# RuyiLian/CheckerPose

Measured on AMD Instinct MI355X. Metric: crops/sec forward (256x256, npt=512), higher is better.
Workload: dtype bf16; 1 GPU; LMO 'ape' hr18GNN2_res6_gnn3Skip_mlpQuery npt=512, PoseNet_GNNskip forward, deterministic random-init weights; global_batch=256, parallelism=dp1 (no forward collective), launch=hipGraph replay of 104 kernel launches

## Files before the change

checkerpose_amd/_abi.py:

```python
import ctypes as C
import os

_HERE = os.path.dirname(os.path.abspath(__file__))
LIB_PATH = os.environ.get("CHECKERPOSE_AMD_LIB") or os.path.join(_HERE, "libcheckerpose_hip.so")

CP_F32, CP_BF16, CP_F16 = 0, 1, 2
ACT_NONE, ACT_RELU, ACT_LEAKY = 0, 1, 2
LOSS_BCE, LOSS_L1 = 0, 1
POSE_ERR_ADD, POSE_ERR_ADI = 1, 2
BOP_ERR_MSSD, BOP_ERR_MSPD, BOP_ERR_PROJ, BOP_MAP_SMALL, BOP_MAP_LARGE = 1, 2, 4, 16, 32
BOP_MATCH_NO_LDS, BOP_MATCH_SCRATCH_MASK, BOP_SCORES_NO_LDS = 1, 2, 1


class CpConvDesc(C.Structure):
    _fields_ = [("dtype", C.c_int32), ("out_f32", C.c_int32), ("B", C.c_int32), ("H", C.c_int32), ("W", C.c_int32),
                ("Cin", C.c_int32), ("in_cstride", C.c_int32), ("in_coff", C.c_int32),
                ("R", C.c_int32), ("S", C.c_int32), ("stride", C.c_int32), ("pad", C.c_int32),
                ("Ho", C.c_int32), ("Wo", C.c_int32), ("Cout", C.c_int32), ("act", C.c_int32), ("slope", C.c_float), ("ksplit", C.c_int32),
                ("o_base", C.c_int64), ("o_sb", C.c_int64), ("o_sy", C.c_int64), ("o_sx", C.c_int64),
                ("o_sc", C.c_int64)]


_P, _I, _F, _L = C.c_void_p, C.c_int, C.c_float, C.c_longlong

# ... 71 lines not shown
    "cp_device_status": (_I, [_P, _I]),
    "cp_set_deterministic": (None, [_I]),
    "cp_get_deterministic": (_I, []),
    "cp_strerror": (C.c_char_p, [_I]),
    "cp_last_kernel": (C.c_char_p, []),
    "cp_kernel_log_begin": (None, []),
    "cp_kernel_log": (C.c_char_p, []),
    "cp_chan_align": (_I, [_I]),
    "cp_packed_weight_bytes": (C.c_size_t, [_I, _I, _I, _I, _I]),
    "cp_pack_conv_weight": (_I, [_P, _I, _P, _I, _I, _I, _I, _I, _I, _I, _P, _I, _P]),
    "cp_conv2d_igemm": (_I, [_P, C.POINTER(CpConvDesc), _P, _P, _P, _P, _P, _P]),
    "cp_conv2d_igemm_splitk": (_I, [_I, C.c_longlong, _I, _I]),
    "cp_packed_halo_weight_bytes": (C.c_size_t, [_I, _I, _I]),
    "cp_pack_conv3x3_halo_weight": (_I, [_P, _I, _P, _I, _I, _I, _P]),
    "cp_conv3x3_halo": (_I, [_P, C.POINTER(CpConvDesc), _P, _P, _P, _P, _P, _P]),
    "cp_conv2x2_halo_supported": (_I, [_I, _I, _I, _I]),
    "cp_packed_conv2x2_halo_weight_bytes": (C.c_size_t, [_I, _I, _I]),
    "cp_pack_conv2x2_halo_weight": (_I, [_P, _I, _P, _I, _I, _I, _P]),
    "cp_conv2x2_halo": (_I, [_P, C.POINTER(CpConvDesc), _P, _P, _P, _P, _P, _P]),
    "cp_conv3x3_s2_small_supported": (_I, [_I, _I, _I, _I]),
    "cp_conv3x3_s2_small_weight_bytes": (C.c_size_t, [_I, _I]),
    "cp_pack_conv3x3_s2_small_weight": (_I, [_P, _P, _I, _I, _I, _I, _P]),
    "cp_conv3x3_s2_small": (_I, [_P, C.POINTER(CpConvDesc), _P, _P, _P, _P, _P]),
    "cp_conv3x3_halo_up2x_supported": (_I, [_I, _I]),
    "cp_conv3x3_halo_up2x": (_I, [_P, C.POINTER(CpConvDesc), _P, _P, _P, _P, _P]),
    "cp_conv3x3_halo_seg_supported": (_I, [_I, _I, _I]),
    "cp_conv3x3_halo_seg": (_I, [_P, C.POINTER(CpConvDesc), _P, _P, _P, _P, _P, _P, _P, _I, _P]),
    "cp_pack_conv3x3_rows_weight": (_I, [_P, _I, _P, _I, _I, _I, _P]),
    "cp_basicblock_fused": (_I, [_P, C.POINTER(CpConvDesc), _P, _P, _P, _P, _P, _P, _P, _P]),
    "cp_bottleneck_fused": (_I, [_P, C.POINTER(CpConvDesc)] + [_P] * 14),
# ... 236 lines not shown
```

checkerpose_amd/csrc/api.hip:

```cpp
#include <stdarg.h>
#include <stdio.h>
#include <string.h>

#include "common.h"

extern "C" int cp_version(void) { return 218; }

std::atomic<int> g_cp_deterministic{0};
extern "C" void cp_set_deterministic(int on) { g_cp_deterministic.store(on ? 1 : 0, std::memory_order_relaxed); }
extern "C" int cp_get_deterministic(void) { return g_cp_deterministic.load(std::memory_order_relaxed); }

static std::atomic<uint32_t*> g_status_word[256];
uint32_t* cp_status_word(bool create) {
  const int dev = cp_current_device();
  if (dev < 0 || dev > 255) return nullptr;
  uint32_t* p = g_status_word[dev].load(std::memory_order_acquire);
  if (p || !create) return p;
  hipStreamCaptureStatus cs = hipStreamCaptureStatusNone;
  if (hipStreamIsCapturing(nullptr, &cs) == hipSuccess && cs != hipStreamCaptureStatusNone) return nullptr;
  uint32_t* q = nullptr;
  if (hipMalloc((void**)&q, 256) != hipSuccess) return nullptr;
  if (hipMemset(q, 0, 256) != hipSuccess) { (void)hipFree(q); return nullptr; }
  uint32_t* expect = nullptr;
  if (!g_status_word[dev].compare_exchange_strong(expect, q, std::memory_order_acq_rel)) { (void)hipFree(q); return expect; }
// ... 69 lines not shown
```

checkerpose_amd/csrc/conv3x3_halo.hip:

```cpp
#include <stdlib.h>

#include "common.h"
#include <cstring>

struct HaloParams {
  const void* in; const void* w; const float* scale; const float* shift; const void* res; void* out;
  int B, H, W, Cin, in_cs, in_coff, nchunk, Cout, ngroups, NB;
  int tiles_x, tiles_y, total_tiles;
  int act; float slope;
  uint32_t in_bytes, w_bytes;
  long long o_base, o_sb, o_sy, o_sx;
  int Hs, Ws; float up_sy, up_sx;
  const float* seg_w; const float* seg_b; float* seg_out; int seg_S;
};

constexpr int HTH = 8, HTW = 16, HPW = HTW + 2, HPH = HTH + 2, HNPIX = 192;
constexpr int HPLANE = HNPIX * 16, HBUF = 4 * HPLANE;
constexpr int USRH = 7, USRW = 11, USPIX = 80, USBUF = USPIX * 64;

template <typename Tag> struct MmaH;
template <> struct MmaH<F32Tag> {
  static __device__ __forceinline__ void run(const u32x4& w, const u32x4& a, f32x4& acc) {
    acc = __builtin_amdgcn_mfma_f32_16x16x4f32(__uint_as_float(w.x), __uint_as_float(a.x), acc, 0, 0, 0);
    acc = __builtin_amdgcn_mfma_f32_16x16x4f32(__uint_as_float(w.y), __uint_as_float(a.y), acc, 0, 0, 0);
// ... 518 lines not shown
  const int lane = (int)((i / E) % 64);
  size_t blk = i / (E * 64);
  const int nt = (int)(blk % 4); blk /= 4;
  const int tap = (int)(blk % 9); blk /= 9;
  const int c = (int)(blk % nchunk);
  const int g = (int)(blk / nchunk);
  const int row = lane & 15, kq = lane >> 4;
  const int n = g * 64 + (row >> 2) * 16 + nt * 4 + (row & 3);
  const int cin = c * (4 * E) + kq * E + e;
  float v = 0.f;
  if (n < Cout && cin < Cin) v = w[((size_t)n * Cin + cin) * 9 + tap];
  store_elem<Tag>(out, i, v);
}

static inline bool halo_wide(int Cout) { return Cout >= 256 && Cout % 256 == 0 && !cp_knob("CP_NO_HALO4"); }

template <typename Tag, int NT, int KS = 3>
__global__ __launch_bounds__(256) void conv3x3_halo_s_kernel(const HaloParams p) {
  if (KS == 2 && p.seg_S == CP_F16) cp_f16_saturate_on();
  constexpr int E = Tag::E;
  constexpr int KCH = 4 * E;
  constexpr int ES = 16 / E;
  constexpr int NTAP = KS * KS;
  constexpr int WPIECES = NTAP * NT * 64;
  constexpr int WITER = (WPIECES + 255) / 256;
  extern __shared__ __attribute__((aligned(16))) unsigned char smem[];
  unsigned char* const sA = smem;
  unsigned char* const sW = smem + HBUF;

  const int t = blockIdx.x;
// ... 632 lines not shown
    } else {
      if (residual) CP_LAUNCH((conv3x3_halo4_kernel<BF16Tag, true, false, false>), dim3(grid4), dim3(256), 2 * HBUF, st4, p);
      else CP_LAUNCH((conv3x3_halo4_kernel<BF16Tag, false, false, false>), dim3(grid4), dim3(256), 2 * HBUF, st4, p);
    }
    return cp_check_launch();
  }
  const unsigned grid = (unsigned)(((tt + 7) / 8) * 8 * p.NB);
  hipStream_t st = (hipStream_t)stream;
  if (d->dtype == CP_F32) {
    if (residual) CP_LAUNCH((conv3x3_halo_kernel<F32Tag, true>), dim3(grid), dim3(256), 2 * HBUF, st, p);
    else CP_LAUNCH((conv3x3_halo_kernel<F32Tag, false>), dim3(grid), dim3(256), 2 * HBUF, st, p);
  } else {
    if (residual) CP_LAUNCH((conv3x3_halo_kernel<BF16Tag, true>), dim3(grid), dim3(256), 2 * HBUF, st, p);
    else CP_LAUNCH((conv3x3_halo_kernel<BF16Tag, false>), dim3(grid), dim3(256), 2 * HBUF, st, p);
  }
  return cp_check_launch();
}

extern "C" int cp_conv3x3_halo_up2x_supported(int dtype, int Cout) {
  return (dtype == CP_F32 || dtype == CP_BF16) && halo_wide(Cout) ? 1 : 0;
}

extern "C" int cp_conv3x3_halo_up2x(cp_stream_t stream, const CpConvDesc* d, const void* in, const void* packed_w,
                                    const float* scale, const float* shift, void* out) {
  if (!d || !in || !packed_w || !scale || !shift || !out) return CP_ERR_INVALID;
  if (!cp_conv3x3_halo_up2x_supported(d->dtype, d->Cout) || !cp_act_ok(d->act, d->slope)) return CP_ERR_INVALID;
  if (d->R != 3 || d->S != 3 || d->stride != 1 || d->pad != 1 || d->Ho != d->H || d->Wo != d->W || d->out_f32 || d->o_sc != 1)
    return CP_ERR_INVALID;
  if (d->B <= 0 || d->H < 2 || d->W < 2 || (d->H & 1) || (d->W & 1)) return CP_ERR_INVALID;
  const int E = cp_chan_align(d->dtype), es = cp_elem_size(d->dtype);
// ... 196 lines not shown
```

checkerpose_amd/engine.py:

```python
import ctypes as C
import os

import torch

from . import _abi
from ._abi import ACT_LEAKY, ACT_NONE, ACT_RELU, CP_BF16, CP_F16, CP_F32, CpChainTail, CpChainTailConv, CpConvDesc, CpFuseConv

_TORCH_DT = {CP_F32: torch.float32, CP_BF16: torch.bfloat16}
USE_HALO = os.environ.get("CHECKERPOSE_AMD_HALO", "1") != "0"
USE_FUSED_BN = os.environ.get("CHECKERPOSE_AMD_FUSED_BN", "1") != "0"
USE_FUSED_BB = os.environ.get("CHECKERPOSE_AMD_FUSED_BB", "1") != "0"
USE_GEMM = os.environ.get("CHECKERPOSE_AMD_GEMM", "1") != "0"
USE_CHAIN = os.environ.get("CHECKERPOSE_AMD_CHAIN", "1") != "0"
USE_UP_FUSED = os.environ.get("CHECKERPOSE_AMD_UP_FUSED", "1") != "0"
USE_FUSE_OUT = os.environ.get("CHECKERPOSE_AMD_FUSE_OUT", "1") != "0"
USE_S2_SMALL = os.environ.get("CHECKERPOSE_AMD_S2_SMALL", "1") != "0"
USE_SEG_FUSED = os.environ.get("CHECKERPOSE_AMD_SEG_FUSED", "1") != "0"
USE_HALO2 = os.environ.get("CHECKERPOSE_AMD_HALO2", "1") != "0"
USE_CHAIN_TAILS = os.environ.get("CHECKERPOSE_AMD_CHAIN_TAILS", "1") != "0"
USE_CHAIN_TAIL = os.environ.get("CHECKERPOSE_AMD_CHAIN_TAIL", "1") != "0"
FUSE_OUT_MIN_BATCH = int(os.environ.get("CHECKERPOSE_AMD_FUSE_OUT_MIN_BATCH", "1"))
USE_MLP_FUSED = os.environ.get("CHECKERPOSE_AMD_MLP_FUSED", "1") != "0"
MLP_FUSED_MIN_ROWS = int(os.environ.get("CHECKERPOSE_AMD_MLP_FUSED_MIN_ROWS", "1"))
EDGE_SCHED = os.environ.get("CHECKERPOSE_AMD_EDGE_SCHED", "1") != "0"
USE_SPLITK = os.environ.get("CHECKERPOSE_AMD_SPLITK", "1") != "0"
GEMM_WS_SMALL_K = os.environ.get("CHECKERPOSE_AMD_GEMM_WS_SMALL_K", "1") != "0"
USE_MLP_GATHER = os.environ.get("CHECKERPOSE_AMD_MLP_GATHER", "1") != "0"
USE_PATCH_GATHER = os.environ.get("CHECKERPOSE_AMD_PATCH_GATHER", "1") != "0"
USE_STEM = os.environ.get("CHECKERPOSE_AMD_STEM", "1") != "0"
STEM_MIN_BATCH = int(os.environ.get("CHECKERPOSE_AMD_STEM_MIN_BATCH", "96"))
USE_EDGE_FUSED = os.environ.get("CHECKERPOSE_AMD_EDGE_FUSED", "1") != "0"
USE_GNN_F16 = os.environ.get("CHECKERPOSE_AMD_GNN_F16", "1") != "0"
# ... 258 lines not shown
            raise RuntimeError("conv %s: weight expects %d input channels, activation has %d" % (wkey, wCin, x.C))
        halo = (USE_HALO and R == 3 and S == 3 and stride == 1 and pad == 1 and ostr is None and not out_f32
                and not transposed and row_map is None and x.W >= 16 and x.H >= 8 and not (out_half or in_half))
        cdt = CP_F16 if in_half else self.dtype
        if halo and wCout <= 80 and self.dtype == CP_F32:
            halo = _rup(x.Cphys, 16) <= 1.15 * x.Cphys
        kmin = 16 * self.E if not (self.dtype == CP_BF16 and residual is None and x.B * x.H * x.W >= 16384 and GEMM_WS_SMALL_K) else 64
        gemm = (USE_GEMM and R == 1 and S == 1 and stride == 1 and pad == 0 and ostr is None and not out_f32
                and not transposed and row_map is None and wCout >= 96 and x.Cphys >= kmin and not out_half)
        s2small = (USE_S2_SMALL and self.dtype == CP_BF16 and R == 3 and S == 3 and stride == 2 and pad == 1 and ostr is None and not out_f32
                   and not transposed and row_map is None and residual is None and x.H % 2 == 0 and x.W % 2 == 0 and x.B >= self.chain_min
                   and not (out_half or in_half) and bool(self.lib.cp_conv3x3_s2_small_supported(x.H, x.W, x.Cphys, _rup(wCout, self.E))))
        halo2 = (USE_HALO2 and self.dtype == CP_BF16 and R == 2 and S == 2 and stride == 1 and pad == 1 and ostr is None and not out_f32
                 and not transposed and row_map is None and not in_half and not self.ws.repacks_every_step
                 and bool(self.lib.cp_conv2x2_halo_supported(self.dtype, x.H, x.W, _rup(wCout, self.E))))
        if (self.splitk and not transposed and row_map is None and (halo or gemm or s2small or halo2)
                and self.lib.cp_conv2d_igemm_splitk(cdt, x.B * ((x.H + 2 * pad - R) // stride + 1) * ((x.W + 2 * pad - S) // stride + 1),
                                                    R * S * x.Cphys, _rup(wCout, self.E))):
            halo = gemm = s2small = halo2 = False
        if s2small:
            ck = ("s2small", wkey, x.Cphys)
            if ck not in self.ws.cache:
                buf = torch.empty(self.lib.cp_conv3x3_s2_small_weight_bytes(x.Cphys, _rup(wCout, self.E)), dtype=torch.uint8, device=self.device)
                wc = w.contiguous()
                self.ws.keep.append(wc)
                st_ = torch.cuda.current_stream(self.device).cuda_stream
                _abi.check(self.lib.cp_pack_conv3x3_s2_small_weight(st_, wc.data_ptr(), wCout, wCin, x.Cphys, _rup(wCout, self.E), buf.data_ptr()),
                           "cp_pack_conv3x3_s2_small_weight(%s)" % wkey)
                self.ws.cache[ck] = buf
            packed = self.ws.cache[ck]
            halo = gemm = False
        elif halo2:
            ck = ("halo2", wkey, x.Cphys)
            if ck not in self.ws.cache:
                buf = torch.empty(self.lib.cp_packed_conv2x2_halo_weight_bytes(self.dtype, wCout, x.Cphys), dtype=torch.uint8, device=self.device)
                wc = w.contiguous()
                self.ws.keep.append(wc)
                st_ = torch.cuda.current_stream(self.device).cuda_stream
                _abi.check(self.lib.cp_pack_conv2x2_halo_weight(st_, self.dtype, wc.data_ptr(), wCout, wCin, x.Cphys, buf.data_ptr()),
                           "cp_pack_conv2x2_halo_weight(%s)" % wkey)
                self.ws.cache[ck] = buf
            packed = self.ws.cache[ck]
        elif halo:
            packed = self.ws.pack_halo(wkey, w, wCout, wCin, x.Cphys)
        elif gemm:
            packed = self.ws.pack_gemm(wkey, w, wCout, wCin, x.Cphys, **({"dtype": CP_F16} if in_half else {}))
        else:
            packed = self.ws.pack(wkey, w, wCout, wCin, R, S, x.Cphys, rows, transposed, phase, row_map, **({"dtype": CP_F16} if in_half else {}))
        sc, sh = self.ws.affine(wkey + "#" + str(phase), scale, shift, rows)
        Ho, Wo = out_hw if out_hw is not None else ((x.H + 2 * pad - R) // stride + 1, (x.W + 2 * pad - S) // stride + 1)
        d = CpConvDesc()
        d.dtype, d.out_f32 = (CP_F16 if in_half else self.dtype), (1 if out_f32 else (2 if out_half else 0))
        d.B, d.H, d.W = x.B, x.H, x.W
        d.Cin, d.in_cstride, d.in_coff = x.Cphys, x.cstride, x.coff
        d.R, d.S, d.stride, d.pad, d.Ho, d.Wo = R, S, stride, pad, Ho, Wo
        d.act, d.slope = act, slope
        d.ksplit = 0 if self.splitk else -1
        if ostr is None:
# ... 11 lines not shown
        if residual is not None and ostr is None:
            assert (residual.cstride, residual.coff, residual.H, residual.W) == (out.cstride, out.coff, out.H, out.W), \
                "residual must share the output layout"
        fn = self.lib.cp_conv3x3_halo if halo else (self.lib.cp_gemm_rows if gemm else self.lib.cp_conv2d_igemm)
        if halo2:
            fn = self.lib.cp_conv2x2_halo
        dref = C.byref(d)
        pw, ps, pt = packed.data_ptr(), sc.data_ptr(), sh.data_ptr()
        xtb = x.tbuf
        if halo:
            fam = "conv3x3_halo_s" if wCout <= 80 else ("conv3x3_halo4" if wCout % 256 == 0 else "conv3x3_halo")
        else:
            fam = "gemm_rows" if gemm else "conv_igemm"
        if halo2:
            fam = "conv3x3_halo_s"
        if s2small:
            fam = "conv3x3_s2_small"
            self._add(self.lib.cp_conv3x3_s2_small, lambda P: (dref, P(xtb), pw, ps, pt, P(otb)), fam + ":" + wkey, [xtb], [otb])
        else:
            self._add(fn, lambda P: (dref, P(xtb), pw, ps, pt, P(rtb) if rtb is not None else None, P(otb)),
                      fam + ":" + wkey, [xtb, rtb], [otb])
        fl = 2 * x.B * Ho * Wo * R * S * wCin * wCout
        self.flops += fl
        oes = 4 if out_f32 else self.es
        nbytes = (x.B * x.H * x.W * wCin * self.es + x.B * Ho * Wo * wCout * oes * (2 if residual is not None else 1)
                  + R * S * wCin * wCout * self.es)
        self.conv_log.append((wkey, x.B * Ho * Wo, wCout, R * S * wCin, fl, fam, nbytes))
        return out

    def would_splitk(self, M, K, Cout):
        return bool(self.splitk and self.lib.cp_conv2d_igemm_splitk(self.dtype, M, K, _rup(Cout, self.E)))
# ... 16 lines not shown
        d.B, d.H, d.W = x.B, Ho, Wo
        d.Cin, d.in_cstride, d.in_coff = x.Cphys, x.cstride, x.coff
        d.R, d.S, d.stride, d.pad, d.Ho, d.Wo = 3, 3, 1, 1, Ho, Wo
        d.act, d.slope, d.Cout = act, slope, out.Cphys
        d.o_base, d.o_sb, d.o_sy, d.o_sx, d.o_sc = out.coff, out.H * out.W * out.cstride, out.W * out.cstride, out.cstride, 1
        self.keep += [d, packed, sc, sh]
        fn = self.lib.cp_conv3x3_halo_up2x
        dref = C.byref(d)
        pw, ps, pt = packed.data_ptr(), sc.data_ptr(), sh.data_ptr()
        xtb, otb = x.tbuf, out.tbuf
        self._add(fn, lambda P: (dref, P(xtb), pw, ps, pt, P(otb)), "conv3x3_halo4:" + wkey, [xtb], [otb])
        fl = 2 * x.B * Ho * Wo * 9 * wCin * wCout
        self.flops += fl
        nbytes = x.B * x.H * x.W * wCin * self.es + x.B * Ho * Wo * wCout * self.es + 9 * wCin * wCout * self.es
        self.conv_log.append((wkey, x.B * Ho * Wo, wCout, 9 * wCin, fl, "conv3x3_halo4", nbytes))
        return out

    def can_conv_halo_seg(self, x: Act, Cout, S):
        return (USE_SEG_FUSED and USE_HALO and x.W >= 16 and x.H >= 8 and
                bool(self.lib.cp_conv3x3_halo_seg_supported(self.dtype, _rup(Cout, self.E), S)))

    def conv_halo_seg(self, x: Act, wkey, w, scale, shift, act, seg_key, seg_w, seg_b, seg_tbuf, slope=0.0):
        wCout, wCin = w.shape[0], w.shape[1]
        if wCin != x.C:
            raise RuntimeError("conv %s: weight expects %d input channels, activation has %d" % (wkey, wCin, x.C))
        packed = self.ws.pack_halo(wkey, w, wCout, wCin, x.Cphys)
        sc, sh = self.ws.affine(wkey + "#0", scale, shift, wCout)
        S = seg_w.shape[0]
        ck = ("seg_head", seg_key, self.dtype)
        if ck not in self.ws.cache:
# ... 813 lines not shown
```

checkerpose_amd/netbuilder.py:

```python
import os

import torch

from ._abi import ACT_LEAKY, ACT_NONE, ACT_RELU
from .engine import Act, Program, _rup

from .model.backbone import HRNET_CFGS
IMG_FEATS_DIMS = {"resnet34": [64, 128, 256, 512], "hrnet_w18": [128, 256, 512, 1024], "hrnet_w18_small": [128, 256, 512, 1024],
                  "hrnet_w30": [128, 256, 512, 1024]}


FUSE_OUT_DEEP = os.environ.get("CHECKERPOSE_AMD_FUSE_OUT_DEEP", "1") != "0"


DECODER_SPLITK = os.environ.get("CHECKERPOSE_AMD_DECODER_SPLITK", "1") != "0"
HEAD_ON_REFINE_LANE = os.environ.get("CHECKERPOSE_AMD_HEAD_LANE", "1") != "0"
FUSE_SAME_LANE = os.environ.get("CHECKERPOSE_AMD_FUSE_SAME_LANE", "1") != "0"


class NetEmitter:
    def __init__(self, prog: Program, sd):
        self.p, self.ws, self.sd = prog, prog.ws, sd
        self.ones = {}
        self.tp = prog if getattr(prog, "training", False) else None
# ... 532 lines not shown
    bl = em.W(pfx + "mlp.bias")
    if tp is None:
        scv = em._unit(rows)
        shv = torch.cat([bl[:4], torch.zeros(3, device=p.device), bl[4:]]) if r3 else bl
    else:
        scv = tp.const_vec(rows, True)
        shv = tp.live_vec(10, [(0, bl, 0, 4), (7, bl, 4, 3)]) if r3 else tp.live_vec(rows, [(0, bl, 0, rows)])
    p.conv(g, pfx + "mlp", wl.view(nbits, 64, 1, 1), scv, shv,
           1, 1, 1, 0, rows, row_map=rmap, cout_rows=rows, out_f32=True,
           ostr=(0, 13 * N, 0, 1, N), out_tbuf=io["bits_tb"], in_half=(tp is None and p.gnn_half))
    if tp is not None:
        em._out_layer_bwd(pfx + "mlp", wl.view(nbits, 64, 1, 1), g, nbits, io["dinit"], 0, nbits * N, 1, N)
    return g


def _convt_train_tail(em, up, wt, f, o, nf):
    tp = em.tp
    y, st = em._bn_train(o, up + ".1", ACT_RELU, None, None)

    def bwd():
        if y.tbuf not in tp.grads:
            return
        gy = tp.grad_of(y)
        tp.bn_bwd(gy, y, o, st, ACT_RELU, 0.0, None, tp.pg_ptr(up + ".1.weight"), tp.pg_ptr(up + ".1.bias"))
        tp.wgrad(f, gy, tp.pg_ptr(up + ".0.weight"), wt.shape[0], wt.shape[1], 3, 3, 2, 1)
        gf = tp.grad_of(f)
        tp.conv(gy, up + ".0#dgrad", wt, tp.const_vec(wt.shape[0], True), tp.const_vec(wt.shape[0], False), 3, 3, 2, 1,
                wt.shape[0], residual=gf, out=gf)
    tp.tape.append(bwd)
    return y
# ... 84 lines not shown
            s_, t_ = em.ws.bn_fold(bk)
            seg_fused[0] = True
            return p.conv_halo_seg(x, ck, em.W(ck + ".weight"), s_, t_, ACT_RELU, "seg_block", wseg, em.W("seg_block.bias"), io["seg_tb"])
        return em.conv_bn(x, ck, bk, 3, 1, 1, out=out)

    for i in range(active):
        p.set_lane(0)
        up = "up_net.%d" % i
        last = i == active - 1
        if i == 0:
            wt = em.W(up + ".0.weight")
            s, t = em.ws.bn_fold(up + ".1") if tp is None else (None, None)
            o = p.act(2 * f.H, 2 * f.W, nf)
            if tp is not None:
                s, t = tp.const_vec(nf, True), tp.const_vec(nf, False)
            for ph in range(4):
                a, b = ph >> 1, ph & 1
                if tp is None and ph > 0:
                    p.set_lane(2 + ph)
                p.conv(f, up + ".0", wt, s, t, 1 + a, 1 + b, 1, 0, nf, ACT_RELU if tp is None else ACT_NONE, transposed=1, phase=ph,
                       ostr=((a * o.W + b) * o.cstride, o.H * o.W * o.cstride, 2 * o.W * o.cstride, 2 * o.cstride, 1),
                       out_tbuf=o.tbuf, out_hw=(f.H, f.W))
            if tp is None:
                p.set_lane(0)
                for ph in range(1, 4):
                    p.sync(2 + ph, 0)
            if tp is not None:
                o = _convt_train_tail(em, up, wt, f, o, nf)
            f = em.conv_bn(o, up + ".3", up + ".4", 3, 1, 1)
            f = tail_conv(f, up + ".6", up + ".7", last, out=lowcats[1].slice(0, nf) if 1 in lowcats else None)
        elif i in lowcats:
            s1, t1 = em.ws.bn_fold(up + ".2")
            f = p.conv_up2x(lowcats[i], up + ".1", em.W(up + ".1.weight"), s1, t1, ACT_RELU)
            f = tail_conv(f, up + ".4", up + ".5", last, out=lowcats[i + 1].slice(0, nf) if (i + 1) in lowcats else None)
        else:
            sk = feats[-i - 1]
            cat = cats[i] if i in cats else p.act(2 * f.H, 2 * f.W, f.C + sk.C)
            if i == 1 and i in cats:
                p.sync(2, 0)
            p.upsample2x(f, cat.slice(0, f.C))
            if i not in cats:
# ... 173 lines not shown
                and not (DECODER_SPLITK and p.would_splitk(x.B * x.H * x.W, 9 * x.Cphys, em.W(ck + ".weight").shape[0]))):
            s_, t_ = em.ws.bn_fold(bk)
            seg_fused = True
            return p.conv_halo_seg(x, ck, em.W(ck + ".weight"), s_, t_, ACT_RELU, "seg_block", wseg, em.W("seg_block.bias"), io["seg_tb"])
        return em.conv_bn(x, ck, bk, 3, 1, 1, out=out)

    for i in range(active):
        p.set_lane(0)
        up = "up_net.%d" % i
        last = i == active - 1
        nxt = lowcats[i + 1].slice(0, nf) if (i + 1) in lowcats else None
        if i == 0:
            wt = em.W(up + ".0.weight")
            s, t = em.ws.bn_fold(up + ".1") if tp is None else (tp.const_vec(nf, True), tp.const_vec(nf, False))
            o = p.act(2 * f.H, 2 * f.W, nf)
            for ph in range(4):
                a, b = ph >> 1, ph & 1
                if tp is None and ph > 0:
                    p.set_lane(2 + ph)
                p.conv(f, up + ".0", wt, s, t, 1 + a, 1 + b, 1, 0, nf, ACT_RELU if tp is None else ACT_NONE, transposed=1, phase=ph,
                       ostr=((a * o.W + b) * o.cstride, o.H * o.W * o.cstride, 2 * o.W * o.cstride, 2 * o.cstride, 1),
                       out_tbuf=o.tbuf, out_hw=(f.H, f.W))
            if tp is None:
                p.set_lane(0)
                for ph in range(1, 4):
                    p.sync(2 + ph, 0)
            else:
                o = _convt_train_tail(em, up, wt, f, o, nf)
            f = em.conv_bn(o, up + ".3", up + ".4", 3, 1, 1)
            f = tail_conv(f, up + ".6", up + ".7", last, out=nxt)
        elif i in lowcats:
            s1, t1 = em.ws.bn_fold(up + ".2")
            f = p.conv_up2x(lowcats[i], up + ".1", em.W(up + ".1.weight"), s1, t1, ACT_RELU)
            f = tail_conv(f, up + ".4", up + ".5", last, out=nxt)
        else:
            sk = feats[-i - 1]
            cat = cats[i] if i in cats else p.act(2 * f.H, 2 * f.W, f.C + sk.C)
            if i == 1 and i in cats:
                p.sync(2, 0)
            p.upsample2x(f, cat.slice(0, f.C))
            if i not in cats:
                p.upsample2x(sk, cat.slice(f.Cphys, sk.C))
# ... 18 lines not shown
```

include/checkerpose_hip.h:

```cpp
#ifndef CHECKERPOSE_HIP_H
#define CHECKERPOSE_HIP_H

#include <stddef.h>
#include <stdint.h>

#ifdef __cplusplus
extern "C" {
#endif

typedef void* cp_stream_t;

enum { CP_F32 = 0, CP_BF16 = 1, CP_F16 = 2 };
enum { CP_ACT_NONE = 0, CP_ACT_RELU = 1, CP_ACT_LEAKY = 2 };
enum { CP_LOSS_BCE = 0, CP_LOSS_L1 = 1 };
enum {
  CP_OK = 0,
  CP_ERR_INVALID = -1,
  CP_ERR_HIP = -2,
  CP_ERR_ALIGN = -3,
  CP_ERR_RANGE = -4
};

int cp_version(void);
const char* cp_strerror(int code);
// ... 27 lines not shown
  int32_t act;
  float slope;
  int32_t ksplit;
  int64_t o_base, o_sb, o_sy, o_sx, o_sc;
} CpConvDesc;

int cp_conv2d_igemm(cp_stream_t stream, const CpConvDesc* d, const void* in, const void* packed_w,
                    const float* scale, const float* shift, const void* residual, void* out);
int cp_conv2d_igemm_splitk(int dtype, long long M, int K, int Cout);

size_t cp_packed_halo_weight_bytes(int dtype, int Cout, int cin_phys);
int cp_pack_conv3x3_halo_weight(cp_stream_t stream, int dtype, const float* w, int Cout, int Cin, int cin_phys,
                                void* packed);
int cp_conv3x3_halo(cp_stream_t stream, const CpConvDesc* d, const void* in, const void* packed_w,
                    const float* scale, const float* shift, const void* residual, void* out);
int cp_conv2x2_halo_supported(int dtype, int H, int W, int Cout_phys);
size_t cp_packed_conv2x2_halo_weight_bytes(int dtype, int Cout, int Cin_phys);
int cp_pack_conv2x2_halo_weight(cp_stream_t stream, int dtype, const float* w, int Cout, int Cin, int cin_phys, void* packed);
int cp_conv2x2_halo(cp_stream_t stream, const CpConvDesc* d, const void* in, const void* packed_w, const float* scale,
                    const float* shift, const void* residual, void* out);

int cp_conv3x3_halo_up2x_supported(int dtype, int Cout);
int cp_conv3x3_halo_up2x(cp_stream_t stream, const CpConvDesc* d, const void* in, const void* packed_w,
                         const float* scale, const float* shift, void* out);

int cp_conv3x3_halo_seg_supported(int dtype, int Cout, int S);
int cp_conv3x3_halo_seg(cp_stream_t stream, const CpConvDesc* d, const void* in, const void* packed_w, const float* scale,
                        const float* shift, void* out, const float* seg_w, const float* seg_b, int S, float* seg_out);

int cp_conv3x3_s2_small_supported(int H, int W, int cin_phys, int out_cphys);
// ... 511 lines not shown
```

Measured before the change: 26460 crops/s.

## Add paired-crop 8x8 halo conv kernel and single-launch phase-split transposed conv

Adds a specialised 3x3 halo conv kernel for 8x8 bf16 feature maps that processes two crops per block with double-buffered LDS staging and software-pipelined MFMA over taps. It also handles the stride-2 transposed conv by packing per-phase tap subsets and launching all four output phases in one grid, replacing four separate phase launches on parallel lanes with their syncs. The aim is better MFMA utilisation and fewer launches at the low-resolution decoder stages. In exchange it adds a new weight packing layout and a narrow shape-specific path that is enabled by default.

```diff
diff --git a/checkerpose_amd/_abi.py b/checkerpose_amd/_abi.py
--- a/checkerpose_amd/_abi.py
+++ b/checkerpose_amd/_abi.py
@@ -109,6 +109,10 @@
     "cp_packed_halo_weight_bytes": (C.c_size_t, [_I, _I, _I]),
     "cp_pack_conv3x3_halo_weight": (_I, [_P, _I, _P, _I, _I, _I, _P]),
     "cp_conv3x3_halo": (_I, [_P, C.POINTER(CpConvDesc), _P, _P, _P, _P, _P, _P]),
+    "cp_conv3x3_halo_pair_supported": (_I, [_I, _I, _I, _I]),
+    "cp_packed_convt3x3_halo_pair_weight_bytes": (C.c_size_t, [_I, _I, _I]),
+    "cp_pack_convt3x3_halo_pair_weight": (_I, [_P, _I, _P, _I, _I, _I, _P]),
+    "cp_conv3x3_halo_pair": (_I, [_P, C.POINTER(CpConvDesc), _P, _P, _P, _P, _I, _P]),
     "cp_conv2x2_halo_supported": (_I, [_I, _I, _I, _I]),
     "cp_packed_conv2x2_halo_weight_bytes": (C.c_size_t, [_I, _I, _I]),
     "cp_pack_conv2x2_halo_weight": (_I, [_P, _I, _P, _I, _I, _I, _P]),
diff --git a/checkerpose_amd/csrc/api.hip b/checkerpose_amd/csrc/api.hip
--- a/checkerpose_amd/csrc/api.hip
+++ b/checkerpose_amd/csrc/api.hip
@@ -4,7 +4,7 @@
 
 #include "common.h"
 
-extern "C" int cp_version(void) { return 218; }
+extern "C" int cp_version(void) { return 219; }
 
 std::atomic<int> g_cp_deterministic{0};
 extern "C" void cp_set_deterministic(int on) { g_cp_deterministic.store(on ? 1 : 0, std::memory_order_relaxed); }
diff --git a/checkerpose_amd/csrc/conv3x3_halo.hip b/checkerpose_amd/csrc/conv3x3_halo.hip
--- a/checkerpose_amd/csrc/conv3x3_halo.hip
+++ b/checkerpose_amd/csrc/conv3x3_halo.hip
@@ -556,6 +556,174 @@
 }
 
 static inline bool halo_wide(int Cout) { return Cout >= 256 && Cout % 256 == 0 && !cp_knob("CP_NO_HALO4"); }
+
+constexpr int PPW = 10, PBLK = 104, PNPIX = 208;
+constexpr int PPLANE = PNPIX * 16, PBUF = 4 * PPLANE;
+constexpr int tap_count(int m) { int n = 0; for (int t = 0; t < 9; ++t) n += (m >> t) & 1; return n; }
+constexpr int tap_at(int m, int i) { for (int t = 0; t < 9; ++t) if ((m >> t) & 1) { if (i == 0) return t; --i; } return 0; }
+constexpr int phase_taps(int phase) { return phase == 0 ? 0x010 : (phase == 1 ? 0x030 : (phase == 2 ? 0x090 : 0x1B0)); }
+
+template <int TAPS>
+__device__ __forceinline__ void halo4_pair_tile(const HaloParams& p, const int t, const int nblk, const void* wimg, const uint32_t w_bytes,
+                                                const long long o_base, const long long o_sy, const long long o_sx) {
+  constexpr int E = 8, KCH = 32, NTAP = tap_count(TAPS);
+  extern __shared__ __attribute__((aligned(16))) unsigned char smem[];
+  const int tid = threadIdx.x;
+  const int lane = tid & 63;
+  const int wave = __builtin_amdgcn_readfirstlane(tid >> 6);
+  const int x = lane & 15, q = lane >> 4;
+  const int g = nblk * 4 + wave;
+
+  const __amdgpu_buffer_rsrc_t rsrc = __builtin_amdgcn_make_buffer_rsrc(const_cast<void*>(p.in), 0, p.in_bytes, 0x00020000);
+  const __amdgpu_buffer_rsrc_t wrsrc = __builtin_amdgcn_make_buffer_rsrc(const_cast<void*>(wimg), 0, w_bytes, 0x00020000);
+
+  const int pq = tid & 3;
+  uint32_t s_goff[2], s_lds[2];
+#pragma unroll
+  for (int k = 0; k < 2; ++k) {
+    const int pix = (tid + 256 * k) >> 2;
+    const int crop = pix >> 6, py = (pix >> 3) & 7, px = pix & 7;
+    const int bb = 2 * t + crop;
+    s_goff[k] = bb < p.B ? (uint32_t)((bb * 64 + (pix & 63)) * p.in_cs + p.in_coff + pq * E) : 0xFFFFFFFFu;
+    s_lds[k] = (uint32_t)(pq * PPLANE + (crop * PBLK + (py + 1) * PPW + px + 1) * 16);
+  }
+  auto stage_load = [&](u32x4* v, int c) {
+    const int c0 = c * KCH;
+#pragma unroll
+    for (int k = 0; k < 2; ++k) {
+      const bool ok = (s_goff[k] != 0xFFFFFFFFu) & (c0 + pq * E < p.Cin);
+      v[k] = __builtin_bit_cast(u32x4, __builtin_amdgcn_raw_buffer_load_b128(rsrc, ok ? (s_goff[k] + (uint32_t)c0) * 2u : 0x80000000u, 0, 0));
+    }
+  };
+  auto stage_write = [&](const u32x4* v, int buf) {
+#pragma unroll
+    for (int k = 0; k < 2; ++k) *(u32x4*)(smem + buf * PBUF + s_lds[k]) = v[k];
+  };
+
+  f32x4 acc[8][4];
+#pragma unroll
+  for (int mt = 0; mt < 8; ++mt)
+#pragma unroll
+    for (int nt = 0; nt < 4; ++nt) acc[mt][nt] = f32x4{0.f, 0.f, 0.f, 0.f};
+
+  const uint32_t wbase = ((uint32_t)g * p.nchunk * (NTAP * 4u) * 64u + lane) * 16u;
+  auto w_load = [&](u32x4* w, int c, int ti) {
+    const uint32_t off = wbase + ((uint32_t)c * (NTAP * 4u) + (uint32_t)ti * 4u) * 1024u;
+#pragma unroll
+    for (int nt = 0; nt < 4; ++nt) w[nt] = __builtin_bit_cast(u32x4, __builtin_amdgcn_raw_buffer_load_b128(wrsrc, off + nt * 1024u, 0, 0));
+  };
+  const uint32_t a_lane = (uint32_t)(q * PPLANE + (x + (x >= 8 ? PBLK - 8 : 0)) * 16);
+  auto a_load = [&](u32x4* a, int buf, int tap, int half) {
+    const int r = tap / 3, s2 = tap - 3 * r;
+    const unsigned char* base = smem + buf * PBUF + a_lane + ((r + 4 * half) * PPW + s2) * 16;
+#pragma unroll
+    for (int i = 0; i < 4; ++i) a[i] = *(const u32x4*)(base + i * PPW * 16);
+  };
+  auto mma = [&](const u32x4* a, const u32x4* w, int half) {
+#pragma unroll
+    for (int i = 0; i < 4; ++i)
+#pragma unroll
+      for (int nt = 0; nt < 4; ++nt) MmaH<BF16Tag>::run(w[nt], a[i], acc[4 * half + i][nt]);
+  };
+
+  u32x4 sv[2];
+  u32x4 w[2][4], a0[4], a1[4];
+  stage_load(sv, 0);
+  w_load(w[0], 0, 0);
+  for (int i = tid; i < 2 * PBUF / 16; i += 256) *(u32x4*)(smem + i * 16) = u32x4{0u, 0u, 0u, 0u};
+  __syncthreads();
+  stage_write(sv, 0);
+  __syncthreads();
+
+  for (int c = 0; c < p.nchunk; ++c) {
+    const int buf = c & 1;
+    stage_load(sv, c + 1);
+    a_load(a0, buf, tap_at(TAPS, 0), 0);
+#pragma unroll
+    for (int i = 0; i < NTAP; ++i) {
+      const bool lastt = i == NTAP - 1;
+      a_load(a1, buf, tap_at(TAPS, i), 1);
+      w_load(w[(i + 1) & 1], lastt ? c + 1 : c, lastt ? 0 : i + 1);
+      __builtin_amdgcn_sched_barrier(0);
+      mma(a0, w[i & 1], 0); __builtin_amdgcn_sched_barrier(0);
+      if (!lastt) a_load(a0, buf, tap_at(TAPS, i + 1), 0);
+      __builtin_amdgcn_sched_barrier(0);
+      mma(a1, w[i & 1], 1); __builtin_amdgcn_sched_barrier(0);
+    }
+    if constexpr (NTAP & 1) {
+#pragma unroll
+      for (int nt = 0; nt < 4; ++nt) w[0][nt] = w[1][nt];
+    }
+    stage_write(sv, buf ^ 1);
+    __syncthreads();
+  }
+
+  const int ch = g * 64 + q * 16;
+  const int b = 2 * t + (x >> 3);
+  if (b >= p.B) return;
+  float sc[16], sh[16];
+#pragma unroll
+  for (int nt = 0; nt < 4; ++nt) {
+    const f32x4 s4 = *(const f32x4*)(p.scale + ch + 4 * nt), t4 = *(const f32x4*)(p.shift + ch + 4 * nt);
+#pragma unroll
+    for (int j = 0; j < 4; ++j) { sc[4 * nt + j] = s4[j]; sh[4 * nt + j] = t4[j]; }
+  }
+  const long long o0 = o_base + (long long)b * p.o_sb + (long long)(x & 7) * o_sx + ch;
+#pragma unroll
+  for (int mt = 0; mt < 8; ++mt) {
+    float v[16];
+#pragma unroll
+    for (int nt = 0; nt < 4; ++nt)
+#pragma unroll
+      for (int j = 0; j < 4; ++j) v[4 * nt + j] = cp_act_apply(acc[mt][nt][j] * sc[4 * nt + j] + sh[4 * nt + j], cp_act_slope(p.act, p.slope));
+    uint16_t* const o = (uint16_t*)p.out + o0 + (long long)mt * o_sy;
+    *(u32x4*)o = Vec16<BF16Tag>::pack(v);
+    *(u32x4*)(o + 8) = Vec16<BF16Tag>::pack(v + 8);
+  }
+}
+
+__global__ __launch_bounds__(256, 2) void conv3x3_halo4_pair_kernel(const HaloParams p) {
+  const int t = blockIdx.x / p.NB;
+  halo4_pair_tile<0x1FF>(p, t, blockIdx.x - t * p.NB, p.w, p.w_bytes, p.o_base, p.o_sy, p.o_sx);
+}
+
+__global__ __launch_bounds__(256, 2) void convt3x3_halo4_pair_kernel(const HaloParams p) {
+  const int per = p.total_tiles * p.NB;
+  const int slot = blockIdx.x / per, rem = blockIdx.x - slot * per;
+  const int t = rem / p.NB, nblk = rem - t * p.NB;
+  const unsigned char* const w = (const unsigned char*)p.w;
+  const long long sy = 2 * p.o_sy, sx = 2 * p.o_sx;
+  switch (slot) {
+    case 0: halo4_pair_tile<phase_taps(3)>(p, t, nblk, w + 5ull * p.w_bytes, 4u * p.w_bytes, p.o_base + p.o_sy + p.o_sx, sy, sx); break;
+    case 1: halo4_pair_tile<phase_taps(1)>(p, t, nblk, w + 1ull * p.w_bytes, 2u * p.w_bytes, p.o_base + p.o_sx, sy, sx); break;
+    case 2: halo4_pair_tile<phase_taps(2)>(p, t, nblk, w + 3ull * p.w_bytes, 2u * p.w_bytes, p.o_base + p.o_sy, sy, sx); break;
+    default: halo4_pair_tile<phase_taps(0)>(p, t, nblk, w, p.w_bytes, p.o_base, sy, sx); break;
+  }
+}
+
+template <typename Tag>
+__global__ void pack_halo4_taps_weight_kernel(const float* __restrict__ w, void* __restrict__ out, int Cout, int Cin, int nchunk,
+                                              int taps, int ntap, int pa, int pb, size_t total) {
+  constexpr int E = Tag::E;
+  const size_t i = (size_t)blockIdx.x * blockDim.x + threadIdx.x;
+  if (i >= total) return;
+  const int e = (int)(i % E);
+  const int lane = (int)((i / E) % 64);
+  size_t blk = i / (E * 64);
+  const int nt = (int)(blk % 4); blk /= 4;
+  const int tap = tap_at(taps, (int)(blk % ntap)); blk /= ntap;
+  const int c = (int)(blk % nchunk);
+  const int g = (int)(blk / nchunk);
+  const int row = lane & 15, kq = lane >> 4;
+  const int n = g * 64 + (row >> 2) * 16 + nt * 4 + (row & 3);
+  const int cin = c * (4 * E) + kq * E + e;
+  float v = 0.f;
+  if (n < Cout && cin < Cin) {
+    const int r = tap / 3, s = tap - 3 * r;
+    v = w[((size_t)cin * Cout + n) * 9 + (pa + 3 - 2 * r) * 3 + (pb + 3 - 2 * s)];
+  }
+  store_elem<Tag>(out, i, v);
+}
 
 template <typename Tag, int NT, int KS = 3>
 __global__ __launch_bounds__(256) void conv3x3_halo_s_kernel(const HaloParams p) {
@@ -1218,6 +1386,63 @@
     if (residual) CP_LAUNCH((conv3x3_halo_kernel<BF16Tag, true>), dim3(grid), dim3(256), 2 * HBUF, st, p);
     else CP_LAUNCH((conv3x3_halo_kernel<BF16Tag, false>), dim3(grid), dim3(256), 2 * HBUF, st, p);
   }
+  return cp_check_launch();
+}
+
+extern "C" int cp_conv3x3_halo_pair_supported(int dtype, int H, int W, int Cout) {
+  return dtype == CP_BF16 && H == 8 && W == 8 && halo_wide(Cout) ? 1 : 0;
+}
+
+static inline size_t pair_tap_bytes(int Cout, int cin_phys) { return (size_t)(Cout / 64) * (((size_t)cin_phys + 31) / 32) * 4 * 1024; }
+
+extern "C" size_t cp_packed_convt3x3_halo_pair_weight_bytes(int dtype, int Cout, int cin_phys) {
+  if (dtype != CP_BF16 || Cout <= 0 || Cout % 64 || cin_phys <= 0) return 0;
+  return 9 * pair_tap_bytes(Cout, cin_phys);
+}
+
+extern "C" int cp_pack_convt3x3_halo_pair_weight(cp_stream_t stream, int dtype, const float* w, int Cout, int Cin, int cin_phys, void* packed) {
+  if (!w || !packed || Cout <= 0 || Cin <= 0 || cin_phys < Cin) return CP_ERR_INVALID;
+  if (dtype != CP_BF16 || Cout % 64) return CP_ERR_INVALID;
+  if (cin_phys % 8 || !cp_aligned16(packed)) return CP_ERR_ALIGN;
+  const size_t share = pair_tap_bytes(Cout, cin_phys);
+  size_t off = 0;
+  for (int phase = 0; phase < 4; ++phase) {
+    const int taps = phase_taps(phase), ntap = tap_count(taps);
+    const size_t total = share * ntap / 2;
+    CP_LAUNCH(pack_halo4_taps_weight_kernel<BF16Tag>, dim3((unsigned)((total + 255) / 256)), dim3(256), 0, (hipStream_t)stream, w,
+              (unsigned char*)packed + off, Cout, Cin, (cin_phys + 31) / 32, taps, ntap, phase >> 1, phase & 1, total);
+    off += share * ntap;
+  }
+  return cp_check_launch();
+}
+
+extern "C" int cp_conv3x3_halo_pair(cp_stream_t stream, const CpConvDesc* d, const void* in, const void* packed_w,
+                                    const float* scale, const float* shift, int transposed, void* out) {
+  if (!d || !in || !packed_w || !scale || !shift || !out) return CP_ERR_INVALID;
+  if ((transposed != 0 && transposed != 1) || !cp_act_ok(d->act, d->slope)) return CP_ERR_INVALID;
+  if (!cp_conv3x3_halo_pair_supported(d->dtype, d->H, d->W, d->Cout) || d->B <= 0 || d->out_f32 || d->o_sc != 1) return CP_ERR_INVALID;
+  if (d->R != 3 || d->S != 3 || d->pad != 1 || d->stride != 1 + transposed || d->Ho != d->H * d->stride || d->Wo != d->W * d->stride)
+    return CP_ERR_INVALID;
+  if (d->Cin <= 0 || d->Cin % 8 || d->in_coff % 8 || d->in_cstride % 8 || d->in_coff + d->Cin > d->in_cstride) return CP_ERR_ALIGN;
+  if (!cp_aligned16(in) || !cp_aligned16(packed_w) || !cp_aligned16(scale) || !cp_aligned16(shift) || !cp_aligned16(out)) return CP_ERR_ALIGN;
+  if ((d->o_base % 8) || (d->o_sb % 8) || (d->o_sy % 8) || (d->o_sx % 8)) return CP_ERR_ALIGN;
+  const long long in_bytes = (long long)d->B * 64 * d->in_cstride * 2;
+  if (in_bytes >= (1LL << 31)) return CP_ERR_RANGE;
+  const size_t wb = transposed ? pair_tap_bytes(d->Cout, d->Cin) : cp_packed_halo_weight_bytes(d->dtype, d->Cout, d->Cin);
+  if (wb >= (1ull << (transposed ? 29 : 31))) return CP_ERR_RANGE;
+  HaloParams p;
+  memset(&p, 0, sizeof(p));
+  p.in = in; p.w = packed_w; p.scale = scale; p.shift = shift; p.out = out;
+  p.B = d->B; p.H = d->H; p.W = d->W; p.Cin = d->Cin; p.in_cs = d->in_cstride; p.in_coff = d->in_coff;
+  p.nchunk = (d->Cin + 31) / 32;
+  p.Cout = d->Cout; p.ngroups = d->Cout / 32; p.NB = d->Cout / 256;
+  p.tiles_x = p.tiles_y = 1; p.total_tiles = (d->B + 1) / 2;
+  p.act = d->act; p.slope = d->slope;
+  p.in_bytes = (uint32_t)in_bytes; p.w_bytes = (uint32_t)wb;
+  p.o_base = d->o_base; p.o_sb = d->o_sb; p.o_sy = d->o_sy; p.o_sx = d->o_sx;
+  const unsigned grid = (unsigned)p.total_tiles * p.NB;
+  if (transposed) CP_LAUNCH(convt3x3_halo4_pair_kernel, dim3(4 * grid), dim3(256), 2 * PBUF, (hipStream_t)stream, p);
+  else CP_LAUNCH(conv3x3_halo4_pair_kernel, dim3(grid), dim3(256), 2 * PBUF, (hipStream_t)stream, p);
   return cp_check_launch();
 }
 
diff --git a/checkerpose_amd/engine.py b/checkerpose_amd/engine.py
--- a/checkerpose_amd/engine.py
+++ b/checkerpose_amd/engine.py
@@ -16,6 +16,7 @@
 USE_FUSE_OUT = os.environ.get("CHECKERPOSE_AMD_FUSE_OUT", "1") != "0"
 USE_S2_SMALL = os.environ.get("CHECKERPOSE_AMD_S2_SMALL", "1") != "0"
 USE_SEG_FUSED = os.environ.get("CHECKERPOSE_AMD_SEG_FUSED", "1") != "0"
+USE_HALO_PAIR = os.environ.get("CHECKERPOSE_AMD_HALO_PAIR", "1") != "0"
 USE_HALO2 = os.environ.get("CHECKERPOSE_AMD_HALO2", "1") != "0"
 USE_CHAIN_TAILS = os.environ.get("CHECKERPOSE_AMD_CHAIN_TAILS", "1") != "0"
 USE_CHAIN_TAIL = os.environ.get("CHECKERPOSE_AMD_CHAIN_TAIL", "1") != "0"
@@ -304,6 +305,11 @@
         halo2 = (USE_HALO2 and self.dtype == CP_BF16 and R == 2 and S == 2 and stride == 1 and pad == 1 and ostr is None and not out_f32
                  and not transposed and row_map is None and not in_half and not self.ws.repacks_every_step
                  and bool(self.lib.cp_conv2x2_halo_supported(self.dtype, x.H, x.W, _rup(wCout, self.E))))
+        pair = (USE_HALO_PAIR and USE_HALO and self.dtype == CP_BF16 and not self.ws.repacks_every_step and residual is None and not out_f32
+                and not transposed and row_map is None and not (out_half or in_half) and cout_rows is None and ostr is None
+                and R == 3 and S == 3 and stride == 1 and pad == 1
+                and bool(self.lib.cp_conv3x3_halo_pair_supported(self.dtype, x.H, x.W, _rup(wCout, self.E)))
+                and not (self.splitk and self.lib.cp_conv2d_igemm_splitk(cdt, x.B * x.H * x.W, R * S * x.Cphys, _rup(wCout, self.E))))
         if (self.splitk and not transposed and row_map is None and (halo or gemm or s2small or halo2)
                 and self.lib.cp_conv2d_igemm_splitk(cdt, x.B * ((x.H + 2 * pad - R) // stride + 1) * ((x.W + 2 * pad - S) // stride + 1),
                                                     R * S * x.Cphys, _rup(wCout, self.E))):
@@ -331,7 +337,7 @@
                            "cp_pack_conv2x2_halo_weight(%s)" % wkey)
                 self.ws.cache[ck] = buf
             packed = self.ws.cache[ck]
-        elif halo:
+        elif halo or pair:
             packed = self.ws.pack_halo(wkey, w, wCout, wCin, x.Cphys)
         elif gemm:
             packed = self.ws.pack_gemm(wkey, w, wCout, wCin, x.Cphys, **({"dtype": CP_F16} if in_half else {}))
@@ -373,7 +379,10 @@
             fam = "gemm_rows" if gemm else "conv_igemm"
         if halo2:
             fam = "conv3x3_halo_s"
-        if s2small:
+        if pair:
+            fam = "conv3x3_halo4"
+            self._add(self.lib.cp_conv3x3_halo_pair, lambda P: (dref, P(xtb), pw, ps, pt, 0, P(otb)), fam + ":" + wkey, [xtb], [otb])
+        elif s2small:
             fam = "conv3x3_s2_small"
             self._add(self.lib.cp_conv3x3_s2_small, lambda P: (dref, P(xtb), pw, ps, pt, P(otb)), fam + ":" + wkey, [xtb], [otb])
         else:
@@ -420,6 +429,47 @@
         self.flops += fl
         nbytes = x.B * x.H * x.W * wCin * self.es + x.B * Ho * Wo * wCout * self.es + 9 * wCin * wCout * self.es
         self.conv_log.append((wkey, x.B * Ho * Wo, wCout, 9 * wCin, fl, "conv3x3_halo4", nbytes))
+        return out
+
+    def can_convt_pair(self, x: Act, Cout):
+        return (USE_HALO_PAIR and USE_HALO and self.dtype == CP_BF16 and not self.ws.repacks_every_step
+                and bool(self.lib.cp_conv3x3_halo_pair_supported(self.dtype, x.H, x.W, _rup(Cout, self.E)))
+                and not any(self.would_splitk(x.B * x.H * x.W, k * x.Cphys, Cout) for k in (1, 2, 4)))
+
+    def convt_pair(self, x: Act, wkey, wt, scale, shift, act=ACT_NONE, slope=0.0, out: Act = None):
+        wCin, wCout = wt.shape[0], wt.shape[1]
+        if wCin != x.C:
+            raise RuntimeError("conv %s: weight expects %d input channels, activation has %d" % (wkey, wCin, x.C))
+        ck = ("convt_pair", wkey, x.Cphys)
+        if ck not in self.ws.cache:
+            buf = torch.empty(self.lib.cp_packed_convt3x3_halo_pair_weight_bytes(self.dtype, wCout, x.Cphys), dtype=torch.uint8, device=self.device)
+            wc = wt.contiguous()
+            self.ws.keep.append(wc)
+            st_ = torch.cuda.current_stream(self.device).cuda_stream
+            _abi.check(self.lib.cp_pack_convt3x3_halo_pair_weight(st_, self.dtype, wc.data_ptr(), wCout, wCin, x.Cphys, buf.data_ptr()),
+                       "cp_pack_convt3x3_halo_pair_weight(%s)" % wkey)
+            self.ws.cache[ck] = buf
+        packed = self.ws.cache[ck]
+        sc, sh = self.ws.affine(wkey + "#0", scale, shift, wCout)
+        Ho, Wo = 2 * x.H, 2 * x.W
+        if out is None:
+            out = self.act(Ho, Wo, wCout)
+        d = CpConvDesc()
+        d.dtype, d.out_f32 = self.dtype, 0
+        d.B, d.H, d.W = x.B, x.H, x.W
+        d.Cin, d.in_cstride, d.in_coff = x.Cphys, x.cstride, x.coff
+        d.R, d.S, d.stride, d.pad, d.Ho, d.Wo = 3, 3, 2, 1, Ho, Wo
+        d.act, d.slope, d.Cout = act, slope, out.Cphys
+        d.o_base, d.o_sb, d.o_sy, d.o_sx, d.o_sc = out.coff, out.H * out.W * out.cstride, out.W * out.cstride, out.cstride, 1
+        self.keep += [d, packed, sc, sh]
+        dref = C.byref(d)
+        pw, ps, pt = packed.data_ptr(), sc.data_ptr(), sh.data_ptr()
+        xtb, otb = x.tbuf, out.tbuf
+        self._add(self.lib.cp_conv3x3_halo_pair, lambda P: (dref, P(xtb), pw, ps, pt, 1, P(otb)), "conv3x3_halo4:" + wkey, [xtb], [otb])
+        fl = 2 * x.B * x.H * x.W * 9 * wCin * wCout
+        self.flops += fl
+        nbytes = x.B * x.H * x.W * wCin * self.es + x.B * Ho * Wo * wCout * self.es + 9 * wCin * wCout * self.es
+        self.conv_log.append((wkey, x.B * Ho * Wo, wCout, 9 * wCin // 4, fl, "conv3x3_halo4", nbytes))
         return out
 
     def can_conv_halo_seg(self, x: Act, Cout, S):
diff --git a/checkerpose_amd/netbuilder.py b/checkerpose_amd/netbuilder.py
--- a/checkerpose_amd/netbuilder.py
+++ b/checkerpose_amd/netbuilder.py
@@ -570,6 +570,23 @@
     return g
 
 
+def _convt_entry(p, tp, up, wt, s, t, f, o, nf):
+    if tp is None and p.can_convt_pair(f, nf):
+        p.convt_pair(f, up + ".0", wt, s, t, ACT_RELU, out=o)
+        return
+    for ph in range(4):
+        a, b = ph >> 1, ph & 1
+        if tp is None and ph > 0:
+            p.set_lane(2 + ph)
+        p.conv(f, up + ".0", wt, s, t, 1 + a, 1 + b, 1, 0, nf, ACT_RELU if tp is None else ACT_NONE, transposed=1, phase=ph,
+               ostr=((a * o.W + b) * o.cstride, o.H * o.W * o.cstride, 2 * o.W * o.cstride, 2 * o.cstride, 1),
+               out_tbuf=o.tbuf, out_hw=(f.H, f.W))
+    if tp is None:
+        p.set_lane(0)
+        for ph in range(1, 4):
+            p.sync(2 + ph, 0)
+
+
 def _convt_train_tail(em, up, wt, f, o, nf):
     tp = em.tp
     y, st = em._bn_train(o, up + ".1", ACT_RELU, None, None)
@@ -684,17 +701,7 @@
             o = p.act(2 * f.H, 2 * f.W, nf)
             if tp is not None:
                 s, t = tp.const_vec(nf, True), tp.const_vec(nf, False)
-            for ph in range(4):
-                a, b = ph >> 1, ph & 1
-                if tp is None and ph > 0:
-                    p.set_lane(2 + ph)
-                p.conv(f, up + ".0", wt, s, t, 1 + a, 1 + b, 1, 0, nf, ACT_RELU if tp is None else ACT_NONE, transposed=1, phase=ph,
-                       ostr=((a * o.W + b) * o.cstride, o.H * o.W * o.cstride, 2 * o.W * o.cstride, 2 * o.cstride, 1),
-                       out_tbuf=o.tbuf, out_hw=(f.H, f.W))
-            if tp is None:
-                p.set_lane(0)
-                for ph in range(1, 4):
-                    p.sync(2 + ph, 0)
+            _convt_entry(p, tp, up, wt, s, t, f, o, nf)
             if tp is not None:
                 o = _convt_train_tail(em, up, wt, f, o, nf)
             f = em.conv_bn(o, up + ".3", up + ".4", 3, 1, 1)
@@ -898,18 +905,8 @@
             wt = em.W(up + ".0.weight")
             s, t = em.ws.bn_fold(up + ".1") if tp is None else (tp.const_vec(nf, True), tp.const_vec(nf, False))
             o = p.act(2 * f.H, 2 * f.W, nf)
-            for ph in range(4):
-                a, b = ph >> 1, ph & 1
-                if tp is None and ph > 0:
-                    p.set_lane(2 + ph)
-                p.conv(f, up + ".0", wt, s, t, 1 + a, 1 + b, 1, 0, nf, ACT_RELU if tp is None else ACT_NONE, transposed=1, phase=ph,
-                       ostr=((a * o.W + b) * o.cstride, o.H * o.W * o.cstride, 2 * o.W * o.cstride, 2 * o.cstride, 1),
-                       out_tbuf=o.tbuf, out_hw=(f.H, f.W))
-            if tp is None:
-                p.set_lane(0)
-                for ph in range(1, 4):
-                    p.sync(2 + ph, 0)
-            else:
+            _convt_entry(p, tp, up, wt, s, t, f, o, nf)
+            if tp is not None:
                 o = _convt_train_tail(em, up, wt, f, o, nf)
             f = em.conv_bn(o, up + ".3", up + ".4", 3, 1, 1)
             f = tail_conv(f, up + ".6", up + ".7", last, out=nxt)
diff --git a/include/checkerpose_hip.h b/include/checkerpose_hip.h
--- a/include/checkerpose_hip.h
+++ b/include/checkerpose_hip.h
@@ -65,6 +65,11 @@
                                 void* packed);
 int cp_conv3x3_halo(cp_stream_t stream, const CpConvDesc* d, const void* in, const void* packed_w,
                     const float* scale, const float* shift, const void* residual, void* out);
+int cp_conv3x3_halo_pair_supported(int dtype, int H, int W, int Cout);
+size_t cp_packed_convt3x3_halo_pair_weight_bytes(int dtype, int Cout, int cin_phys);
+int cp_pack_convt3x3_halo_pair_weight(cp_stream_t stream, int dtype, const float* w, int Cout, int Cin, int cin_phys, void* packed);
+int cp_conv3x3_halo_pair(cp_stream_t stream, const CpConvDesc* d, const void* in, const void* packed_w, const float* scale,
+                         const float* shift, int transposed, void* out);
 int cp_conv2x2_halo_supported(int dtype, int H, int W, int Cout_phys);
 size_t cp_packed_conv2x2_halo_weight_bytes(int dtype, int Cout, int Cin_phys);
 int cp_pack_conv2x2_halo_weight(cp_stream_t stream, int dtype, const float* w, int Cout, int Cin, int cin_phys, void* packed);
```

Measured after the change: 25640 crops/s. 0.969x the previous value.
